# someone-in-somewhere/multimodal_rag

Hardware: AMD Instinct MI355X
Metric: chunks embedded/sec + queries/sec top_k=5 over 1M×768 at 1/2/4/8 GPUs (higher is better)
Workload: dtype f16

## Files before the change

### include/mmrag.h

```cpp
#ifndef MMRAG_H
#define MMRAG_H

#include <stddef.h>
#include <stdint.h>

#ifdef __cplusplus
extern "C" {
#endif

#define MMRAG_OK 0
#define MMRAG_EINVAL 1
#define MMRAG_EWORKSPACE 2
#define MMRAG_EHIP 3
#define MMRAG_EUNSUPPORTED 4

#define MMRAG_F32 0
#define MMRAG_F16 1
#define MMRAG_BF16 2
#define MMRAG_F8E4M3 3

#define MMRAG_MAX_K 20

int mmrag_abi_version(void);
const char *mmrag_last_error(void);

int64_t mmrag_padded_dim(int d, int dtype);

size_t mmrag_cosine_topk_workspace_bytes(int B, int64_t n, int k);

int mmrag_cosine_topk(const void *q, const void *corpus, int B, int64_t n, int d, int64_t ld,
                      int dtype, int k, int64_t row_offset, const uint32_t *alive_bits,
                      float *out_scores, int64_t *out_rows, void *workspace,
                      size_t workspace_bytes, void *stream);

int mmrag_cosine_topk_lists(const void *q, const void *corpus, int B, int64_t n, int d, int64_t ld,
                            int dtype, int k, const uint32_t *alive_bits, void *workspace,
                            size_t workspace_bytes, void *stream);
int mmrag_cosine_topk_select(int B, int64_t n, int k, int64_t row_offset, const void *workspace,
                             float *out_scores, int64_t *out_rows, void *stream);

#define MMRAG_MAX_K_DEEP 4096
size_t mmrag_cosine_topk_deep_workspace_bytes(int B, int64_t n, int k);
int mmrag_cosine_topk_deep(const void *q, const void *corpus, int B, int64_t n, int d, int64_t ld,
                           int dtype, int k, int64_t row_offset, const uint32_t *alive_bits,
                           float *out_scores, int64_t *out_rows, void *workspace,
                           size_t workspace_bytes, void *stream);

#define MMRAG_MAX_RESCORE_CANDIDATES 4096
int mmrag_rescore_topk(const void *q, const void *plane, int64_t ld, int dtype, int d, const int64_t *cand_rows,
                       int B, int C, int k, float *out_scores, int64_t *out_rows, void *stream);

int mmrag_merge_topk(const float *scores, const int64_t *rows, int G, int B, int k_in, int k,
                     float *out_scores, int64_t *out_rows, void *stream);
int mmrag_merge_topk_host(const float *scores, const int64_t *rows, int G, int B, int k_in,
                          int k, float *out_scores, int64_t *out_rows);
int mmrag_merge_topk_host_packed(const void *blocks, int G, int B, int k_in, int k,
                                 float *out_scores, int64_t *out_rows);

int mmrag_append_rows(void *corpus, int64_t capacity, int64_t ld, int dtype, int64_t n_used,
                      const float *new_rows, int64_t m, int d, void *stream);

int mmrag_gather_rows(void *dst, const void *src, int64_t ld, int dtype,
// ... 367 lines not shown
```

### multimodal_rag_amd/_native.py

```python
from __future__ import annotations

import ctypes
import os
import threading
from ctypes import c_char_p, c_float, c_int, c_int32, c_int64, c_size_t, c_void_p
from typing import Optional, Tuple

import numpy as np
import torch

_PKG = os.path.dirname(os.path.abspath(__file__))
LIB_PATH = os.path.join(_PKG, "lib", "libmmrag.so")

F32, F16, BF16, F8E4M3 = 0, 1, 2, 3
MAX_K = 20
MAX_K_DEEP = 4096
MAX_MMR_CANDIDATES = 1024
MAX_RESCORE_CANDIDATES = 4096
MAX_GROUP_CANDIDATES, MAX_GROUPS, MAX_GROUP_SIZE = 4096, 256, 16
MAX_FUSE_LISTS, MAX_FUSE_CANDIDATES, MAX_FUSE_RESULTS = 16, 256, 4096
FUSE_METHODS = {"rrf": 0, "max": 1}
MAX_JOIN_PAIRS = 1 << 26
MAX_CLUSTERS = 4096
MAX_SCOPE_GROUPS = 64
# ... 20 lines not shown
    pass


def _declare(lib):
    lib.mmrag_abi_version.restype = c_int
    lib.mmrag_last_error.restype = c_char_p
    lib.mmrag_padded_dim.restype = c_int64
    lib.mmrag_padded_dim.argtypes = [c_int, c_int]
    lib.mmrag_cosine_topk_workspace_bytes.restype = c_size_t
    lib.mmrag_cosine_topk_workspace_bytes.argtypes = [c_int, c_int64, c_int]
    lib.mmrag_cosine_topk.restype = c_int
    lib.mmrag_cosine_topk.argtypes = [c_void_p, c_void_p, c_int, c_int64, c_int, c_int64, c_int, c_int,
                                      c_int64, c_void_p, c_void_p, c_void_p, c_void_p, c_size_t, c_void_p]
    lib.mmrag_cosine_topk_lists.restype = c_int
    lib.mmrag_cosine_topk_lists.argtypes = [c_void_p, c_void_p, c_int, c_int64, c_int, c_int64, c_int, c_int,
                                            c_void_p, c_void_p, c_size_t, c_void_p]
    lib.mmrag_internal_search_uses_qs.restype = c_int
    lib.mmrag_internal_search_uses_qs.argtypes = [c_int, c_int64, c_int64, c_int, c_int]
    lib.mmrag_internal_cosine_topk_lists_ex.restype = c_int
    lib.mmrag_internal_cosine_topk_lists_ex.argtypes = [c_void_p, c_void_p, c_int, c_int64, c_int, c_int64, c_int,
                                                        c_int, c_void_p, c_void_p, c_size_t, c_void_p, ctypes.c_uint]
    lib.mmrag_cosine_topk_select.restype = c_int
    lib.mmrag_cosine_topk_select.argtypes = [c_int, c_int64, c_int, c_int64, c_void_p, c_void_p, c_void_p, c_void_p]
    lib.mmrag_cosine_topk_deep_workspace_bytes.restype = c_size_t
    lib.mmrag_cosine_topk_deep_workspace_bytes.argtypes = [c_int, c_int64, c_int]
    lib.mmrag_cosine_topk_deep.restype = c_int
    lib.mmrag_cosine_topk_deep.argtypes = lib.mmrag_cosine_topk.argtypes
    lib.mmrag_internal_cosine_topk_deep_ex.restype = c_int
    lib.mmrag_internal_cosine_topk_deep_ex.argtypes = lib.mmrag_cosine_topk.argtypes + [ctypes.c_uint, c_int64]
    lib.mmrag_rescore_topk.restype = c_int
    lib.mmrag_rescore_topk.argtypes = [c_void_p, c_void_p, c_int64, c_int, c_int, c_void_p, c_int, c_int, c_int,
                                       c_void_p, c_void_p, c_void_p]
    lib.mmrag_merge_topk.restype = c_int
    lib.mmrag_merge_topk.argtypes = [c_void_p, c_void_p, c_int, c_int, c_int, c_int, c_void_p, c_void_p, c_void_p]
    lib.mmrag_merge_topk_host.restype = c_int
    lib.mmrag_merge_topk_host.argtypes = [c_void_p, c_void_p, c_int, c_int, c_int, c_int, c_void_p, c_void_p]
    lib.mmrag_merge_topk_host_packed.restype = c_int
    lib.mmrag_merge_topk_host_packed.argtypes = [c_void_p, c_int, c_int, c_int, c_int, c_void_p, c_void_p]
    lib.mmrag_append_rows.restype = c_int
    lib.mmrag_append_rows.argtypes = [c_void_p, c_int64, c_int64, c_int, c_int64, c_void_p, c_int64, c_int, c_void_p]
    lib.mmrag_gather_rows.restype = c_int
    lib.mmrag_gather_rows.argtypes = [c_void_p, c_void_p, c_int64, c_int, c_void_p, c_int64, c_void_p]
    lib.mmrag_fetch_rows_f32.restype = c_int
    lib.mmrag_fetch_rows_f32.argtypes = [c_void_p, c_int64, c_int, c_void_p, c_int64, c_int, c_void_p, c_void_p]
    lib.mmrag_device_info.restype = c_int
    lib.mmrag_device_info.argtypes = [ctypes.POINTER(c_int), ctypes.POINTER(c_int), ctypes.POINTER(c_int64)]
# ... 321 lines not shown
    return buf[B * k * 8:].view(torch.float32).view(B, k), buf[: B * k * 8].view(torch.int64).view(B, k)


def search_uses_query_stationary(B: int, n: int, d: int, k: int, dtype: torch.dtype) -> bool:
    return bool(lib().mmrag_internal_search_uses_qs(B, n, padded_dim(d, dtype), _TORCH2DT[dtype], k))


def search_kernel_name(B: int, n: int, d: int, k: int, dtype: torch.dtype) -> str:
    v = lib().mmrag_internal_search_uses_qs(B, n, padded_dim(d, dtype), _TORCH2DT[dtype], k)
    return {0: "cosine_topk_kernel (slab-ring)", 1: "cosine_topk_qs_kernel", 2: "cosine_topk_walk_kernel"}[v]


def padded_dim(d: int, dtype: torch.dtype) -> int:
    v = lib().mmrag_padded_dim(int(d), _TORCH2DT[dtype])
    if v < 0:
        raise MMRagNativeError(f"padded_dim: bad arguments d={d} dtype={dtype}")
    return int(v)


DBG_NO_PREPASS, DBG_8_WAVES, DBG_NO_QS, DBG_FORCE_QS = 1, 2, 4, 8
DBG_OLD_QS, DBG_MFMA32, DBG_MFMA16, DBG_NO_DYN, DBG_NO_SEED = 0x10000, 0x20000, 0x40000, 0x80000, 0x100000


def cosine_topk(q: torch.Tensor, corpus: torch.Tensor, n: int, d: int, k: int, row_offset: int = 0,
                alive_bits: Optional[torch.Tensor] = None,
                workspace: Optional[torch.Tensor] = None, dbg: int = 0,
                packed_out: bool = False) -> Tuple[torch.Tensor, torch.Tensor]:
    _dev_check(q, corpus, alive_bits)
    _check_q_rows("cosine_topk", q, corpus, n)
    B, ld = q.shape
    L = lib()
    need = L.mmrag_cosine_topk_workspace_bytes(B, n, k)
    if workspace is None or _nbytes(workspace) < need:
        workspace = torch.empty(max(need, 16), dtype=torch.uint8, device=q.device)
    out_s, out_r = _topk_out(B, k, q.device, packed_out)
    if dbg:
        cosine_topk_lists(q, corpus, n, d, k, workspace, alive_bits=alive_bits, dbg=dbg)
        return cosine_topk_select(B, n, k, row_offset, workspace, out_s, out_r)
    with torch.cuda.device(q.device):
        st = L.mmrag_cosine_topk(q.data_ptr(), corpus.data_ptr(), B, n, d, ld, _TORCH2DT[q.dtype], k, row_offset,
                                 alive_bits.data_ptr() if alive_bits is not None else None,
                                 out_s.data_ptr(), out_r.data_ptr(), workspace.data_ptr(), _nbytes(workspace),
                                 _stream_ptr(q.device))
    _check(st, "mmrag_cosine_topk")
    return out_s, out_r


DEEP_DBG_NO_BOUND = 1


def cosine_topk_deep(q: torch.Tensor, corpus: torch.Tensor, n: int, d: int, k: int, row_offset: int = 0,
                     alive_bits: Optional[torch.Tensor] = None, workspace: Optional[torch.Tensor] = None,
                     dbg: int = 0, cap: int = 0) -> Tuple[torch.Tensor, torch.Tensor]:
    _dev_check(q, corpus, alive_bits)
    _check_q_rows("cosine_topk_deep", q, corpus, n)
    B, ld = q.shape
    L = lib()
    need = cosine_topk_deep_workspace_bytes(B, n, k)
    if workspace is None or _nbytes(workspace) < need:
        workspace = torch.empty(max(need, 16), dtype=torch.uint8, device=q.device)
    out_s, out_r = _topk_out(B, k, q.device)
# ... 1191 lines not shown
    with torch.cuda.device(corpus.device):
        st = lib().mmrag_fetch_rows_f32(corpus.data_ptr(), corpus.shape[1], _TORCH2DT[corpus.dtype], rows.data_ptr(),
                                        rows.numel(), d, out.data_ptr(), _stream_ptr(corpus.device))
    _check(st, "mmrag_fetch_rows_f32")
    return out


def cosine_topk_lists(q: torch.Tensor, corpus: torch.Tensor, n: int, d: int, k: int, workspace: torch.Tensor,
                      alive_bits: Optional[torch.Tensor] = None, dbg: int = 0) -> None:
    _dev_check(q, corpus, workspace, alive_bits)
    if q.dtype != corpus.dtype or q.shape[1] != corpus.shape[1] or not q.is_contiguous() or not corpus.is_contiguous():
        raise MMRagNativeError("cosine_topk_lists: q and corpus must be contiguous and share dtype and padded width")
    if n > corpus.shape[0]:
        raise MMRagNativeError(f"cosine_topk_lists: n={n} exceeds corpus capacity {corpus.shape[0]}")
    B, ld = q.shape
    with torch.cuda.device(q.device):
        st = lib().mmrag_internal_cosine_topk_lists_ex(
            q.data_ptr(), corpus.data_ptr(), B, n, d, ld, _TORCH2DT[q.dtype], k,
            alive_bits.data_ptr() if alive_bits is not None else None, workspace.data_ptr(),
            _nbytes(workspace), _stream_ptr(q.device), int(dbg))
    _check(st, "mmrag_cosine_topk_lists")


def cosine_topk_select(B: int, n: int, k: int, row_offset: int, workspace: torch.Tensor,
                       out_scores: Optional[torch.Tensor] = None,
                       out_rows: Optional[torch.Tensor] = None) -> Tuple[torch.Tensor, torch.Tensor]:
    _dev_check(workspace)
    dev = workspace.device
    if out_scores is None:
        out_scores = torch.empty((B, k), dtype=torch.float32, device=dev)
    if out_rows is None:
        out_rows = torch.empty((B, k), dtype=torch.int64, device=dev)
    with torch.cuda.device(dev):
        st = lib().mmrag_cosine_topk_select(B, n, k, row_offset, workspace.data_ptr(), out_scores.data_ptr(),
                                            out_rows.data_ptr(), _stream_ptr(dev))
    _check(st, "mmrag_cosine_topk_select")
    return out_scores, out_rows


ACT_NONE, ACT_GELU, ACT_QUICK_GELU = 0, 1, 2
ARCH_BERT, ARCH_PRELN = 0, 1
POOL_MEAN, POOL_FIRST, POOL_SELECT = 0, 1, 2


class EncoderDesc(ctypes.Structure):
    _fields_ = [("arch", c_int32), ("n_layers", c_int32), ("hidden", c_int32), ("n_heads", c_int32),
                ("intermediate", c_int32), ("vocab", c_int32), ("max_pos", c_int32), ("pool", c_int32),
                ("act", c_int32), ("causal", c_int32), ("normalize", c_int32), ("out_dim", c_int32),
                ("ln_eps", c_float), ("image", c_int32), ("patch", c_int32)]


def _ptr(t: Optional[torch.Tensor]):
    return t.data_ptr() if t is not None else None


def linear_f16(x: torch.Tensor, wt: torch.Tensor, bias: Optional[torch.Tensor] = None, act: int = ACT_NONE,
               resid: Optional[torch.Tensor] = None, out: Optional[torch.Tensor] = None) -> torch.Tensor:
    _dev_check(x, wt, bias, resid, out)
# ... 561 lines not shown
        raise MMRagNativeError("copy_to_host_async: need a host destination at least as large as the device source")
    _check(lib().mmrag_copy_to_host_async(dst_host.data_ptr(), src_dev.data_ptr(), nbytes, stream),
           "mmrag_copy_to_host_async")


class SearchPlan:

    def __init__(self, q: torch.Tensor, corpus: torch.Tensor, n: int, d: int, k: int, workspace: torch.Tensor,
                 alive_bits: Optional[torch.Tensor] = None):
        _dev_check(q, corpus, workspace, alive_bits)
        if q.dtype != corpus.dtype or q.shape[1] != corpus.shape[1] or not q.is_contiguous() or not corpus.is_contiguous():
            raise MMRagNativeError("SearchPlan: q and corpus must be contiguous and share dtype and padded width")
        if n > corpus.shape[0]:
            raise MMRagNativeError(f"SearchPlan: n={n} exceeds corpus capacity {corpus.shape[0]}")
        need = lib().mmrag_cosine_topk_workspace_bytes(q.shape[0], n, k)
        if _nbytes(workspace) < need:
            raise MMRagNativeError("SearchPlan: workspace too small")
        self._keep = (q, corpus, workspace, alive_bits)
        self.B, self.n, self.k = q.shape[0], n, k
        self._scan_args = (q.data_ptr(), corpus.data_ptr(), q.shape[0], n, d, q.shape[1], _TORCH2DT[q.dtype], k,
                           alive_bits.data_ptr() if alive_bits is not None else None, workspace.data_ptr(),
                           _nbytes(workspace))
        self._ws = workspace.data_ptr()
        self._scan = lib().mmrag_cosine_topk_lists
        self._select = lib().mmrag_cosine_topk_select

    def scan(self, stream: int) -> None:
        st = self._scan(*self._scan_args, stream)
        if st:
            _check(st, "mmrag_cosine_topk_lists")

    def select(self, row_offset: int, out_scores_ptr: int, out_rows_ptr: int, stream: int) -> None:
        st = self._select(self.B, self.n, self.k, row_offset, self._ws, out_scores_ptr, out_rows_ptr, stream)
        if st:
            _check(st, "mmrag_cosine_topk_select")
```

### multimodal_rag_amd/csrc/search.hip

```cpp
#include "slab_ring.h"

#include <stdlib.h>

using namespace mmrag;

namespace mmrag_impl {

template <int DT, int WN, int K, int NSTAGE, int NW, bool SEEDED>
__global__ __launch_bounds__(64 * NW, NW / 4) void cosine_topk_kernel(const KParams p) {
#if defined(__HIP_DEVICE_COMPILE__)
#include "slab_ring_body.inc"
#endif
}

template <int K>
struct FullList {
    float v[K];
    long long r[K];
    __device__ inline void init() {
#pragma unroll
        for (int i = 0; i < K; ++i) {
            v[i] = NEG_INF;
            r[i] = LLONG_MAX;
        }
    }
    __device__ inline void insert(float x, long long xr) {
#pragma unroll
        for (int j = 0; j < K; ++j) {
            const bool b = better(x, xr, v[j], r[j]);
            const float nv = b ? x : v[j];
            const float nx = b ? v[j] : x;
            const long long nr = b ? xr : r[j];
            const long long nxr = b ? r[j] : xr;
            v[j] = nv;
            x = nx;
            r[j] = nr;
            xr = nxr;
        }
    }
    __device__ inline void pop() {
#pragma unroll
        for (int j = 0; j + 1 < K; ++j) {
            v[j] = v[j + 1];
            r[j] = r[j + 1];
        }
        v[K - 1] = NEG_INF;
        r[K - 1] = LLONG_MAX;
    }
};

template <int K>
__device__ inline void wave_extract(FullList<K> &l, float *out_v, long long *out_r) {
#pragma unroll
    for (int round = 0; round < K; ++round) {
        float s = l.v[0];
        long long r = l.r[0];
#pragma unroll
        for (int off = 32; off >= 1; off >>= 1) {
            const float os = __shfl_xor(s, off);
            const long long orr = __shfl_xor(r, off);
            if (better(os, orr, s, r)) {
                s = os;
                r = orr;
            }
        }
        out_v[round] = s;
        out_r[round] = r;
        if (l.v[0] == s && l.r[0] == r) l.pop();
    }
}
// ... 39 lines not shown
        for (int i = lane; i < 4 * K; i += 64)
            if (sh_r[i] != LLONG_MAX) l.insert(sh_v[i], sh_r[i]);
        wave_extract<K>(l, ov, orr);
        if (lane == 0) {
#pragma unroll
            for (int i = 0; i < K; ++i) {
                if (i < k_out) {
                    const bool valid = orr[i] != LLONG_MAX && ov[i] > NEG_INF;
                    out_s[(size_t)q * k_out + i] = valid ? ov[i] : NEG_INF;
                    out_r[(size_t)q * k_out + i] = valid ? orr[i] + row_offset : -1;
                }
            }
            if (thr0 != nullptr) {
                const bool full = orr[K - 1] != LLONG_MAX && ov[K - 1] > NEG_INF;
                thr0[q] = full ? ov[K - 1] : NEG_INF;
#pragma unroll
                for (int i = 0; i < K; ++i) {
                    const bool valid = orr[i] != LLONG_MAX && ov[i] > NEG_INF;
                    seed_s[(size_t)q * seed_q_stride + i] = valid ? ov[i] : NEG_INF;
                    seed_r[(size_t)q * seed_q_stride + i] = valid ? (int)orr[i] : INT_MAX;
                }
            }
        }
    }
}

struct Plan {
    int K;
    int WN;
    int NW;
    int grid_x, grid_y;
    int n_tiles;
    int n_lists;
    int b_pad;
    int pre_tiles;
    bool qs_ok;
    bool qs_room;
};

constexpr unsigned DBG_NO_PREPASS = 1u, DBG_8_WAVES = 2u, DBG_NO_QS = 4u, DBG_FORCE_QS = 8u;
constexpr unsigned DBG_OLD_QS = 0x10000u, DBG_MFMA32 = 0x20000u, DBG_MFMA16 = 0x40000u, DBG_NO_DYN = 0x80000u,
                   DBG_NO_SEED = 0x100000u;

Plan make_plan(int B, long long n, int k, unsigned dbg = 0) {
    Plan pl;
    pl.K = k <= 5 ? 5 : (k <= 10 ? 10 : 20);
// ... 62 lines not shown
    const dim3 grid(grid_x, grid_y);
    with_elem_type(dtype, [&](auto tag) { launch_filter<decltype(tag)::value>(WN, p, grid, s); });
    MMRAG_CHECK_HIP(hipGetLastError());
    return MMRAG_OK;
}

template <typename RowT>
int launch_merge(int K, const float *cs, const RowT *cr, long long n_cand, long long inner,
                 long long outer_stride, long long q_stride, int B, int k_out, long long row_offset,
                 float *out_s, long long *out_r, hipStream_t s, float *thr0 = nullptr, float *seed_s = nullptr,
                 int *seed_r = nullptr, long long seed_q_stride = 0) {
    if (K == 5)
        merge_topk_kernel<5, RowT><<<B, 256, 0, s>>>(cs, cr, n_cand, inner, outer_stride, q_stride, k_out,
                                                     row_offset, out_s, out_r, thr0, seed_s, seed_r, seed_q_stride);
    else if (K == 10)
        merge_topk_kernel<10, RowT><<<B, 256, 0, s>>>(cs, cr, n_cand, inner, outer_stride, q_stride, k_out,
                                                      row_offset, out_s, out_r, thr0, seed_s, seed_r, seed_q_stride);
    else
        merge_topk_kernel<20, RowT><<<B, 256, 0, s>>>(cs, cr, n_cand, inner, outer_stride, q_stride, k_out,
                                                      row_offset, out_s, out_r, thr0, seed_s, seed_r, seed_q_stride);
    return MMRAG_OK;
}

__global__ void fill_empty_kernel(float *s, long long *r, long long total) {
    const long long i = (long long)blockIdx.x * blockDim.x + threadIdx.x;
    if (i < total) {
        s[i] = NEG_INF;
        r[i] = -1;
    }
}

__global__ void fill_seed_empty_kernel(float *s, int *r, long long q_stride, int K, long long n_queries) {
    const long long q = (long long)blockIdx.x * blockDim.x + threadIdx.x;
    if (q < n_queries)
        for (int i = 0; i < K; ++i) {
            s[q * q_stride + i] = NEG_INF;
            r[q * q_stride + i] = INT_MAX;
        }
}

int check_search_args(const char *name, int k_max, const void *q, const void *corpus, int B, int64_t n, int d, int64_t ld,
                      int dtype, int k) {
    MMRAG_CHECK_ARG(dtype >= 0 && dtype <= MMRAG_F8E4M3, "%s: bad dtype %d", name, dtype);
    MMRAG_CHECK_ARG(B > 0, "%s: B must be positive (got %d)", name, B);
    MMRAG_CHECK_ARG(k >= 1 && k <= k_max, "%s: k=%d outside 1..%d", name, k, k_max);
    MMRAG_CHECK_ARG(n >= 0 && n < (int64_t)INT_MAX - TM, "%s: n=%lld out of range", name, (long long)n);
// ... 14 lines not shown

extern "C" {

struct WsLayout {
    size_t entries, off_r, off_thr, off_ts, off_tr, off_cnt, cnt_bytes, off_pub, off_pthr, off_tk, xch_end, total;
};
static WsLayout ws_layout(const Plan &pl) {
    WsLayout w;
    w.entries = (size_t)pl.b_pad * pl.n_lists * pl.K;
    w.off_r = w.entries * sizeof(float);
    w.off_thr = w.off_r + w.entries * sizeof(int);
    w.off_ts = w.off_thr + (size_t)pl.b_pad * sizeof(float);
    w.off_tr = (w.off_ts + (size_t)pl.b_pad * pl.K * sizeof(float) + 15) / 16 * 16;
    w.off_cnt = (w.off_tr + (size_t)pl.b_pad * pl.K * sizeof(long long) + 63) / 64 * 64;
    w.cnt_bytes = 0;
    w.off_pub = w.off_cnt + w.cnt_bytes;
    w.off_pthr = w.off_pub + (pl.qs_room ? (size_t)pl.b_pad * pl.grid_x * sizeof(float) : 0);
    w.off_tk = w.off_pthr + (pl.qs_room ? (size_t)pl.b_pad * sizeof(float) : 0);
    w.xch_end = w.off_tk + (pl.qs_room ? ((size_t)pl.grid_y * sizeof(unsigned) + 63) / 64 * 64 : 0);
    w.total = w.xch_end;
    return w;
}

size_t mmrag_cosine_topk_workspace_bytes(int B, int64_t n, int k) {
    if (B <= 0 || n < 0 || k < 1 || k > MMRAG_MAX_K) return 0;
    return ws_layout(make_plan(B, n, k)).total + 256;
}

int mmrag_internal_cosine_topk_lists_ex(const void *q, const void *corpus, int B, int64_t n, int d, int64_t ld,
                                        int dtype, int k, const uint32_t *alive_bits, void *workspace,
                                        size_t workspace_bytes, void *stream, unsigned dbg) {
    if (int st = check_search_args("cosine_topk", MMRAG_MAX_K, q, corpus, B, n, d, ld, dtype, k)) return st;
    if (n == 0) return MMRAG_OK;
    const Plan pl = make_plan(B, n, k, dbg);
    const WsLayout wl = ws_layout(pl);
    if (!workspace || workspace_bytes < wl.total) {
        set_error("cosine_topk: workspace %zu bytes < required %zu", workspace_bytes, wl.total);
        return MMRAG_EWORKSPACE;
    }
    MMRAG_CHECK_ARG(((uintptr_t)workspace % 16) == 0, "cosine_topk: workspace must be 16-byte aligned");

    KParams p;
    p.q = (const char *)q;
    p.corpus = (const char *)corpus;
    p.alive_bits = alive_bits;
    p.cand_s = (float *)workspace;
    p.cand_r = (int *)((char *)workspace + wl.off_r);
    p.n = n;
    p.B = B;
    p.row_bytes = (unsigned)(ld * esize(dtype));
    p.n_tiles = pl.n_tiles;
    p.n_lists = pl.n_lists;
    p.tile0 = 0;
    p.thr0 = nullptr;
    p.dbg = dbg;
    p.stamps = ((dbg & DBG_QS_CLOCK) && workspace_bytes >= wl.total + 256 * (size_t)(pl.grid_x * pl.grid_y)) ? (unsigned long long *)((char *)workspace + wl.total) : nullptr;
    p.walkers = pl.grid_x;
    p.share_l2 = pl.grid_y > 1;
    p.sample_best = nullptr;
    p.pub_best = nullptr;
    p.pub_thr = nullptr;
    p.tickets = nullptr;
    p.p_static = INT_MAX / 2;
    hipStream_t s = (hipStream_t)stream;
    const size_t seed_off = (size_t)(pl.n_lists - 1) * pl.K;
    const int walk_mfma = (dbg & DBG_MFMA32) ? 32 : ((dbg & DBG_MFMA16) ? 16 : (pl.K == 5 ? QSW_DEFAULT_MFMA : 32));
    if (pl.qs_ok && !(dbg & DBG_OLD_QS) && qsw_supported(dtype, p.row_bytes, pl.K, walk_mfma)) {
        const int tiles = (int)((n + QS_TILE_ROWS - 1) / QS_TILE_ROWS);
        const int per = tiles / pl.grid_x;
        p.n_tiles = tiles;
        p.pub_best = nullptr;
        p.pub_thr = nullptr;
        p.tickets = nullptr;
        p.p_static = INT_MAX / 2;
        const bool seed = per >= 12 && !(dbg & DBG_NO_SEED);
        const bool dyn = pl.grid_y == 1 && per >= 24 && !(dbg & DBG_NO_DYN);
        if (seed || dyn) {
            MMRAG_CHECK_HIP(hipMemsetD32Async((hipDeviceptr_t)((char *)workspace + wl.off_pub), (int)TICKET0,
                                              (wl.xch_end - wl.off_pub) / 4, s));
            if (seed) {
                p.pub_best = (float *)((char *)workspace + wl.off_pub);
                p.pub_thr = (float *)((char *)workspace + wl.off_pthr);
            }
            if (dyn) {
                p.tickets = (unsigned *)((char *)workspace + wl.off_tk);
                const int tail = per / 10 > 3 ? per / 10 : 3;
                p.p_static = per - tail;
            }
        }
        if (int st = qsw_launch(dtype, pl.K, walk_mfma, p, pl.grid_x, pl.grid_y, s)) return st;
        MMRAG_CHECK_HIP(hipGetLastError());
        return MMRAG_OK;
    }
    if (pl.qs_ok && qs_supported(dtype, p.row_bytes, pl.K)) {
        const int tiles = (int)((n + QS_TILE_ROWS - 1) / QS_TILE_ROWS);
        float *thr0 = nullptr;
        if (pl.pre_tiles > 0) {
            KParams ks = p;
            ks.n_tiles = pl.pre_tiles * (TM / QS_TILE_ROWS);
            ks.sample_best = (float *)((char *)workspace + wl.off_pub);
            if (int st = qs_launch(dtype, pl.K, ks, pl.grid_x, pl.grid_y, s)) return st;
            thr0 = (float *)((char *)workspace + wl.off_thr);
// ... 29 lines not shown
        MMRAG_CHECK_HIP(hipGetLastError());
        if (int st = run(pre, pl.n_tiles - pre, pl.grid_x, thr0)) return st;
    } else {
        if (pl.n_lists > pl.grid_x) {
            const long long total = (long long)pl.b_pad;
            fill_seed_empty_kernel<<<(unsigned)((total + 255) / 256), 256, 0, s>>>(
                p.cand_s + seed_off, p.cand_r + seed_off, (long long)pl.n_lists * pl.K, pl.K, total);
        }
        if (int st = run(0, pl.n_tiles, pl.grid_x, nullptr)) return st;
    }
    MMRAG_CHECK_HIP(hipGetLastError());
    return MMRAG_OK;
}

int mmrag_internal_search_uses_qs(int B, int64_t n, int64_t ld, int dtype, int k) {
    if (B <= 0 || n <= 0 || k <= 0 || k > MMRAG_MAX_K) return 0;
    const Plan pl = make_plan(B, n, k, 0u);
    const unsigned rb = (unsigned)(ld * esize(dtype));
    if (!pl.qs_ok) return 0;
    if (qsw_supported(dtype, rb, pl.K, QSW_DEFAULT_MFMA)) return 2;
    return qs_supported(dtype, rb, pl.K) ? 1 : 0;
}

int mmrag_cosine_topk_lists(const void *q, const void *corpus, int B, int64_t n, int d, int64_t ld, int dtype,
                            int k, const uint32_t *alive_bits, void *workspace, size_t workspace_bytes,
                            void *stream) {
    return mmrag_internal_cosine_topk_lists_ex(q, corpus, B, n, d, ld, dtype, k, alive_bits, workspace,
                                               workspace_bytes, stream, 0u);
}

int mmrag_cosine_topk_select(int B, int64_t n, int k, int64_t row_offset, const void *workspace,
                             float *out_scores, int64_t *out_rows, void *stream) {
    MMRAG_CHECK_ARG(B > 0 && n >= 0 && k >= 1 && k <= MMRAG_MAX_K, "cosine_topk_select: bad shape");
    MMRAG_CHECK_ARG(out_scores && out_rows, "cosine_topk_select: null output");
    hipStream_t s = (hipStream_t)stream;
    if (n == 0) {
        const long long total = (long long)B * k;
        fill_empty_kernel<<<(unsigned)((total + 255) / 256), 256, 0, s>>>(out_scores, (long long *)out_rows, total);
        MMRAG_CHECK_HIP(hipGetLastError());
        return MMRAG_OK;
    }
    MMRAG_CHECK_ARG(workspace, "cosine_topk_select: null workspace");
    const Plan pl = make_plan(B, n, k);
    const WsLayout wl = ws_layout(pl);
    const float *cand_s = (const float *)workspace;
    const int *cand_r = (const int *)((const char *)workspace + wl.off_r);
    const long long n_cand = (long long)pl.n_lists * pl.K;
    launch_merge<int>(pl.K, cand_s, cand_r, n_cand, n_cand, 0, n_cand, B, k, row_offset, out_scores,
                      (long long *)out_rows, s);
    MMRAG_CHECK_HIP(hipGetLastError());
    return MMRAG_OK;
}

int mmrag_cosine_topk(const void *q, const void *corpus, int B, int64_t n, int d, int64_t ld, int dtype,
                      int k, int64_t row_offset, const uint32_t *alive_bits, float *out_scores,
                      int64_t *out_rows, void *workspace, size_t workspace_bytes, void *stream) {
    if (int st = mmrag_cosine_topk_lists(q, corpus, B, n, d, ld, dtype, k, alive_bits, workspace, workspace_bytes,
                                         stream))
        return st;
    return mmrag_cosine_topk_select(B, n, k, row_offset, workspace, out_scores, out_rows, stream);
}

int mmrag_merge_topk(const float *scores, const int64_t *rows, int G, int B, int k_in, int k,
                     float *out_scores, int64_t *out_rows, void *stream) {
    MMRAG_CHECK_ARG(scores && rows && out_scores && out_rows, "merge_topk: null pointer");
    MMRAG_CHECK_ARG(G > 0 && B > 0 && k_in > 0, "merge_topk: bad shape G=%d B=%d k_in=%d", G, B, k_in);
    MMRAG_CHECK_ARG(k >= 1 && k <= MMRAG_MAX_K, "merge_topk: k=%d outside 1..%d", k, MMRAG_MAX_K);
    const int K = k <= 5 ? 5 : (k <= 10 ? 10 : 20);
    launch_merge<long long>(K, scores, (const long long *)rows, (long long)G * k_in, k_in, (long long)B * k_in,
                            k_in, B, k, 0, out_scores, (long long *)out_rows, (hipStream_t)stream);
    MMRAG_CHECK_HIP(hipGetLastError());
    return MMRAG_OK;
}

// ... 2 lines not shown
```

### multimodal_rag_amd/index.py

```python
from __future__ import annotations

import gc
import logging
import operator
import threading
import time
from collections import OrderedDict
from typing import Any, Callable, Dict, List, Optional, Sequence, Tuple

import numpy as np
import torch

from . import _native
from .boost import BoostSpec, check_prior_values
from .filters import ColumnRegistry, names_added_at, pack_programs, try_compile
from .hostutil import load_hostrows
from .tracing import stage

_HOSTROWS = load_hostrows()

logger = logging.getLogger(__name__)


_CMP: Dict[str, Callable[[Any, Any], bool]] = {
# ... 134 lines not shown
        self.name = name
        self.metadata = dict(metadata or {})
        self.dim = int(dim)
        self.dtype = dtype
        self.device = torch.device(device)
        self.ld = _native.padded_dim(self.dim, dtype)
        cap = max(int(capacity), 256)
        self._matrix = self._new_rows(cap, zero=True)
        self.plane_ld = _native.padded_dim(self.dim, rescore_dtype) if rescore_dtype is not None else 0
        self._plane: Optional[torch.Tensor] = None
        if rescore_dtype is not None:
            self._plane = torch.zeros((cap, self.plane_ld), dtype=rescore_dtype, device=self.device)
        self._alive_dev = torch.zeros(self._n_words(cap), dtype=torch.int32, device=self.device)
        self._alive_host = np.zeros(self._n_words(cap), dtype=np.uint32)
        self._n = 0
        self._n_dead = 0
        self._ids: List[Optional[str]] = []
        self._documents: List[Optional[str]] = []
        self._metadatas: List[Dict[str, Any]] = []
        self._meta_index = MetaIndex()
        self._row_of: Dict[str, int] = {}
        self._lock = threading.RLock()
        self._search_ws: Optional[torch.Tensor] = None
        self._deep_ws: Optional[torch.Tensor] = None
        self._scoped_ws: Optional[torch.Tensor] = None
        self._lex = None
        self._sparse = None
        self._pending_sparse = None
        self._groups: Dict[str, Dict[str, Any]] = {}
        self._boosted_ws: Optional[torch.Tensor] = None
        self._recommend_ws: Optional[torch.Tensor] = None
        self._added_at = np.full(cap, np.nan, dtype=np.float64)
        self._priors: Dict[str, Any] = {}
        self._spec_cols: "OrderedDict[Tuple[str, float], Dict[str, Any]]" = OrderedDict()
        self.f32_exact = bool(settings.MMRAG_F32_EXACT_SEARCH)
        self._filter_cols = ColumnRegistry(lambda: (self._metadatas, self._n, self._added_at))
        self._filtered_ws: Optional[torch.Tensor] = None
        self._range_ws: Optional[torch.Tensor] = None
        self.device_filters = bool(settings.MMRAG_DEVICE_FILTERS)
        self._tokens = None
        self._late_ws: Optional[torch.Tensor] = None

    def _new_rows(self, rows: int, zero: bool) -> torch.Tensor:
        make = torch.zeros if zero else torch.empty
        if self.is_f8:
            return make((rows, self.ld), dtype=torch.uint8, device=self.device).view(torch.float8_e4m3fn)
# ... 495 lines not shown
    def _launch_search_rescored(self, query_embeddings, n_results: int, where, check_norm: bool):
        from .config import settings

        qf = self._to_device_f32(query_embeddings, "query", check_norm)
        q8 = self._pack_queries(qf, check_norm=False)
        qp = self._pack_plane_queries(qf)
        bits = self._where_bits(where)
        if n_results <= _native.MAX_K_DEEP:
            C = min(max(_native.MAX_K, int(settings.MMRAG_F8_OVERSAMPLE) * n_results), _native.MAX_K_DEEP)
            C = max(C, n_results)
            _, cand = self._scan(q8, C, bits)
            return _native.rescore_topk(qp, self._plane, self.dim, cand.contiguous(), n_results, packed_out=True)
        scores, rows = self._scan(q8, n_results, bits)
        return _cat_pairs([_native.rescore_topk(qp, self._plane, self.dim, rows[:, i:i + _native.MAX_K].contiguous(),
                                                min(_native.MAX_K, rows.shape[1] - i))
                           for i in range(0, rows.shape[1], _native.MAX_K)], 1)

    def _scan(self, q: torch.Tensor, n_results: int, bits):
        if n_results <= _native.MAX_K and self.f32_exact and self.dtype == torch.float32 and q.shape[0] > 64:
            return self._in_slices(q, 64, lambda qi: _native.cosine_topk(qi, self._matrix, self._n, self.dim, n_results,
                                                                         alive_bits=bits))
        if n_results <= _native.MAX_K:
            need = _native.cosine_topk_workspace_bytes(q.shape[0], self._n, n_results)
            return _native.cosine_topk(q, self._matrix, self._n, self.dim, n_results, alive_bits=bits,
                                       workspace=self._workspace("_search_ws", need), packed_out=True)
        if n_results <= _native.MAX_K_DEEP:
            step = 64 if self.f32_exact and self.dtype == torch.float32 else q.shape[0]

            def deep(qi: torch.Tensor):
                need = _native.cosine_topk_deep_workspace_bytes(qi.shape[0], self._n, n_results)
                return _native.cosine_topk_deep(qi, self._matrix, self._n, self.dim, n_results, alive_bits=bits,
                                                workspace=self._workspace("_deep_ws", need))

            return self._in_slices(q, step, deep)
        if q.shape[0] != 1:
            raise ValueError(f"n_results > {_native.MAX_K_DEEP} is supported for single queries only")
        if bits is None:
            bits = self._alive_dev
        bits = bits.clone()
        out_s, out_r, left = [], [], n_results
        while left > 0:
            k = min(left, _native.MAX_K)
            s, r = _native.cosine_topk(q, self._matrix, self._n, self.dim, k, alive_bits=bits)
            out_s.append(s)
            out_r.append(r)
            got = r[0]
            got = got[got >= 0]
            if got.numel() < k:
                break
            host = got.cpu().numpy()
            w = bits.cpu().numpy().view(np.uint32).copy()
            np.bitwise_and.at(w, host >> 5, ~(np.uint32(1) << (host & 31).astype(np.uint32)))
            bits = torch.from_numpy(w.view(np.int32)).to(self.device)
            left -= k
        return torch.cat(out_s, 1), torch.cat(out_r, 1)

    def _workspace(self, name: str, need: int) -> Optional[torch.Tensor]:
        if torch.cuda.current_stream(self.device) != torch.cuda.default_stream(self.device):
            return None
        ws = getattr(self, name)
        if ws is None or ws.numel() < need:
            ws = torch.empty(max(need, 16), dtype=torch.uint8, device=self.device)
            setattr(self, name, ws)
        return ws

    @staticmethod
    def _in_slices(q: torch.Tensor, step: int, run):
        return _cat_pairs([run(q[i:i + step]) for i in range(0, q.shape[0], step)], 0)

    def search(self, query_embeddings, n_results: int, where: Optional[Dict[str, Any]] = None):
        with self._lock:
            return self._launch_search(query_embeddings, n_results, where)

    def _tables(self):
        return self._ids, self._documents, self._metadatas

    @staticmethod
    def _rows_of(tables, rows: Sequence[int], include: Sequence[str]):
        ids_t, docs_t, metas_t = tables
        return ([ids_t[r] for r in rows],
                [docs_t[r] for r in rows] if "documents" in include else None,
                [dict(metas_t[r]) for r in rows] if "metadatas" in include else None)

    @classmethod
    def _append_hits(cls, out: Dict[str, Any], tables, rows: Sequence[int], include: Sequence[str]):
        for key, col in zip(("ids", "documents", "metadatas"), cls._rows_of(tables, rows, include)):
# ... 1525 lines not shown
```

Before: 692,300.

## Fuse exchange-buffer rearm into new select kernel and skip per-search memset

Adds a dedicated per-query top-k select kernel that uses 32-bit row ids and wave-shuffle reduction, replacing the generic merge launch. It also re-initialises the scan's seed/exchange buffer with ticket values at the end of select. A host-side state token records that the buffer is already armed, so the next scan can skip its hipMemsetD32Async. This removes one memset launch per search and a slower merge, at the cost of host-side state that must be reset whenever the workspace is reallocated or reused by another caller.

```diff
diff --git a/include/mmrag.h b/include/mmrag.h
--- a/include/mmrag.h
+++ b/include/mmrag.h
@@ -38,6 +38,15 @@
                             size_t workspace_bytes, void *stream);
 int mmrag_cosine_topk_select(int B, int64_t n, int k, int64_t row_offset, const void *workspace,
                              float *out_scores, int64_t *out_rows, void *stream);
+
+typedef struct {
+    uint64_t armed;
+} mmrag_scan_state;
+int mmrag_cosine_topk_lists_s(const void *q, const void *corpus, int B, int64_t n, int d, int64_t ld,
+                              int dtype, int k, const uint32_t *alive_bits, void *workspace,
+                              size_t workspace_bytes, mmrag_scan_state *state, void *stream);
+int mmrag_cosine_topk_select_s(int B, int64_t n, int k, int64_t row_offset, void *workspace,
+                               float *out_scores, int64_t *out_rows, mmrag_scan_state *state, void *stream);
 
 #define MMRAG_MAX_K_DEEP 4096
 size_t mmrag_cosine_topk_deep_workspace_bytes(int B, int64_t n, int k);
diff --git a/multimodal_rag_amd/_native.py b/multimodal_rag_amd/_native.py
--- a/multimodal_rag_amd/_native.py
+++ b/multimodal_rag_amd/_native.py
@@ -66,6 +66,18 @@
                                                         c_int, c_void_p, c_void_p, c_size_t, c_void_p, ctypes.c_uint]
     lib.mmrag_cosine_topk_select.restype = c_int
     lib.mmrag_cosine_topk_select.argtypes = [c_int, c_int64, c_int, c_int64, c_void_p, c_void_p, c_void_p, c_void_p]
+    lib.mmrag_cosine_topk_lists_s.restype = c_int
+    lib.mmrag_cosine_topk_lists_s.argtypes = [c_void_p, c_void_p, c_int, c_int64, c_int, c_int64, c_int, c_int,
+                                              c_void_p, c_void_p, c_size_t, c_void_p, c_void_p]
+    lib.mmrag_cosine_topk_select_s.restype = c_int
+    lib.mmrag_cosine_topk_select_s.argtypes = [c_int, c_int64, c_int, c_int64, c_void_p, c_void_p, c_void_p, c_void_p,
+                                               c_void_p]
+    lib.mmrag_internal_cosine_topk_select_ex.restype = c_int
+    lib.mmrag_internal_cosine_topk_select_ex.argtypes = [c_int, c_int64, c_int, c_int64, c_void_p, c_void_p, c_void_p,
+                                                         c_void_p, c_void_p, ctypes.c_uint]
+    lib.mmrag_internal_exchange_range.restype = c_int
+    lib.mmrag_internal_exchange_range.argtypes = [c_int, c_int64, c_int, ctypes.POINTER(c_size_t),
+                                                  ctypes.POINTER(c_size_t)]
     lib.mmrag_cosine_topk_deep_workspace_bytes.restype = c_size_t
     lib.mmrag_cosine_topk_deep_workspace_bytes.argtypes = [c_int, c_int64, c_int]
     lib.mmrag_cosine_topk_deep.restype = c_int
@@ -433,10 +445,24 @@
 DBG_OLD_QS, DBG_MFMA32, DBG_MFMA16, DBG_NO_DYN, DBG_NO_SEED = 0x10000, 0x20000, 0x40000, 0x80000, 0x100000
 
 
+class ScanState(ctypes.Structure):
+    _fields_ = [("armed", ctypes.c_uint64)]
+
+    def reset(self) -> None:
+        self.armed = 0
+
+
+def exchange_range(B: int, n: int, k: int) -> Tuple[int, int]:
+    off, length = c_size_t(0), c_size_t(0)
+    _check(lib().mmrag_internal_exchange_range(B, n, k, ctypes.byref(off), ctypes.byref(length)),
+           "mmrag_internal_exchange_range")
+    return off.value, length.value
+
+
 def cosine_topk(q: torch.Tensor, corpus: torch.Tensor, n: int, d: int, k: int, row_offset: int = 0,
                 alive_bits: Optional[torch.Tensor] = None,
                 workspace: Optional[torch.Tensor] = None, dbg: int = 0,
-                packed_out: bool = False) -> Tuple[torch.Tensor, torch.Tensor]:
+                packed_out: bool = False, state: Optional[ScanState] = None) -> Tuple[torch.Tensor, torch.Tensor]:
     _dev_check(q, corpus, alive_bits)
     _check_q_rows("cosine_topk", q, corpus, n)
     B, ld = q.shape
@@ -444,10 +470,26 @@
     need = L.mmrag_cosine_topk_workspace_bytes(B, n, k)
     if workspace is None or _nbytes(workspace) < need:
         workspace = torch.empty(max(need, 16), dtype=torch.uint8, device=q.device)
+        if state is not None:
+            state.reset()
     out_s, out_r = _topk_out(B, k, q.device, packed_out)
     if dbg:
+        if state is not None:
+            state.reset()
         cosine_topk_lists(q, corpus, n, d, k, workspace, alive_bits=alive_bits, dbg=dbg)
         return cosine_topk_select(B, n, k, row_offset, workspace, out_s, out_r)
+    if state is not None:
+        sp = ctypes.addressof(state)
+        with torch.cuda.device(q.device):
+            stream = _stream_ptr(q.device)
+            st = L.mmrag_cosine_topk_lists_s(q.data_ptr(), corpus.data_ptr(), B, n, d, ld, _TORCH2DT[q.dtype], k,
+                                             alive_bits.data_ptr() if alive_bits is not None else None,
+                                             workspace.data_ptr(), _nbytes(workspace), sp, stream)
+            _check(st, "mmrag_cosine_topk_lists_s")
+            st = L.mmrag_cosine_topk_select_s(B, n, k, row_offset, workspace.data_ptr(), out_s.data_ptr(),
+                                              out_r.data_ptr(), sp, stream)
+        _check(st, "mmrag_cosine_topk_select_s")
+        return out_s, out_r
     with torch.cuda.device(q.device):
         st = L.mmrag_cosine_topk(q.data_ptr(), corpus.data_ptr(), B, n, d, ld, _TORCH2DT[q.dtype], k, row_offset,
                                  alive_bits.data_ptr() if alive_bits is not None else None,
@@ -1685,9 +1727,13 @@
     _check(st, "mmrag_cosine_topk_lists")
 
 
+SELECT_DBG_OLD_MERGE = 1
+
+
 def cosine_topk_select(B: int, n: int, k: int, row_offset: int, workspace: torch.Tensor,
                        out_scores: Optional[torch.Tensor] = None,
-                       out_rows: Optional[torch.Tensor] = None) -> Tuple[torch.Tensor, torch.Tensor]:
+                       out_rows: Optional[torch.Tensor] = None, state: Optional[ScanState] = None,
+                       dbg: int = 0) -> Tuple[torch.Tensor, torch.Tensor]:
     _dev_check(workspace)
     dev = workspace.device
     if out_scores is None:
@@ -1695,8 +1741,9 @@
     if out_rows is None:
         out_rows = torch.empty((B, k), dtype=torch.int64, device=dev)
     with torch.cuda.device(dev):
-        st = lib().mmrag_cosine_topk_select(B, n, k, row_offset, workspace.data_ptr(), out_scores.data_ptr(),
-                                            out_rows.data_ptr(), _stream_ptr(dev))
+        st = lib().mmrag_internal_cosine_topk_select_ex(
+            B, n, k, row_offset, workspace.data_ptr(), out_scores.data_ptr(), out_rows.data_ptr(),
+            ctypes.addressof(state) if state is not None else None, _stream_ptr(dev), int(dbg))
     _check(st, "mmrag_cosine_topk_select")
     return out_scores, out_rows
 
@@ -2304,15 +2351,18 @@
                            alive_bits.data_ptr() if alive_bits is not None else None, workspace.data_ptr(),
                            _nbytes(workspace))
         self._ws = workspace.data_ptr()
-        self._scan = lib().mmrag_cosine_topk_lists
-        self._select = lib().mmrag_cosine_topk_select
+        self.state = ScanState()
+        self._state = ctypes.addressof(self.state)
+        self._scan = lib().mmrag_cosine_topk_lists_s
+        self._select = lib().mmrag_cosine_topk_select_s
 
     def scan(self, stream: int) -> None:
-        st = self._scan(*self._scan_args, stream)
+        st = self._scan(*self._scan_args, self._state, stream)
         if st:
-            _check(st, "mmrag_cosine_topk_lists")
+            _check(st, "mmrag_cosine_topk_lists_s")
 
     def select(self, row_offset: int, out_scores_ptr: int, out_rows_ptr: int, stream: int) -> None:
-        st = self._select(self.B, self.n, self.k, row_offset, self._ws, out_scores_ptr, out_rows_ptr, stream)
+        st = self._select(self.B, self.n, self.k, row_offset, self._ws, out_scores_ptr, out_rows_ptr, self._state,
+                          stream)
         if st:
-            _check(st, "mmrag_cosine_topk_select")
+            _check(st, "mmrag_cosine_topk_select_s")
diff --git a/multimodal_rag_amd/csrc/search.hip b/multimodal_rag_amd/csrc/search.hip
--- a/multimodal_rag_amd/csrc/search.hip
+++ b/multimodal_rag_amd/csrc/search.hip
@@ -13,25 +13,26 @@
 #endif
 }
 
-template <int K>
+template <int K, typename RowT = long long>
 struct FullList {
+    static constexpr RowT PAD = sizeof(RowT) == 4 ? (RowT)INT_MAX : (RowT)LLONG_MAX;
     float v[K];
-    long long r[K];
+    RowT r[K];
     __device__ inline void init() {
 #pragma unroll
         for (int i = 0; i < K; ++i) {
             v[i] = NEG_INF;
-            r[i] = LLONG_MAX;
-        }
-    }
-    __device__ inline void insert(float x, long long xr) {
+            r[i] = PAD;
+        }
+    }
+    __device__ inline void insert(float x, RowT xr) {
 #pragma unroll
         for (int j = 0; j < K; ++j) {
             const bool b = better(x, xr, v[j], r[j]);
             const float nv = b ? x : v[j];
             const float nx = b ? v[j] : x;
-            const long long nr = b ? xr : r[j];
-            const long long nxr = b ? r[j] : xr;
+            const RowT nr = b ? xr : r[j];
+            const RowT nxr = b ? r[j] : xr;
             v[j] = nv;
             x = nx;
             r[j] = nr;
@@ -45,7 +46,7 @@
             r[j] = r[j + 1];
         }
         v[K - 1] = NEG_INF;
-        r[K - 1] = LLONG_MAX;
+        r[K - 1] = PAD;
     }
 };
 
@@ -131,6 +132,71 @@
                 }
             }
         }
+    }
+}
+
+constexpr int SELECT_QPB = 4, SELECT_LOADS = 8;
+
+template <int K>
+__global__ __launch_bounds__(64 * SELECT_QPB) void select_topk_kernel(const float *__restrict__ cs,
+                                                                      const int *__restrict__ cr, int n_cand, int B,
+                                                                      int k_out, long long row_offset,
+                                                                      float *__restrict__ out_s,
+                                                                      long long *__restrict__ out_r,
+                                                                      uint4 *__restrict__ rearm, unsigned rearm_words) {
+    const int lane = threadIdx.x & 63;
+    const int q = blockIdx.x * SELECT_QPB + (threadIdx.x >> 6);
+    if (q < B) {
+        const float *qs = cs + (size_t)q * n_cand;
+        const int *qr = cr + (size_t)q * n_cand;
+        FullList<K, int> l;
+        l.init();
+        for (int c0 = lane; c0 < n_cand; c0 += 64 * SELECT_LOADS) {
+            float s[SELECT_LOADS];
+            int r[SELECT_LOADS];
+#pragma unroll
+            for (int u = 0; u < SELECT_LOADS; ++u) {
+                const int c = c0 + 64 * u;
+                s[u] = c < n_cand ? qs[c] : NEG_INF;
+                r[u] = c < n_cand ? qr[c] : INT_MAX;
+            }
+#pragma unroll
+            for (int u = 0; u < SELECT_LOADS; ++u)
+                if (r[u] != INT_MAX && r[u] >= 0 && better(s[u], r[u], l.v[K - 1], l.r[K - 1])) l.insert(s[u], r[u]);
+        }
+        float my_s = NEG_INF;
+        int my_r = INT_MAX;
+#pragma unroll
+        for (int round = 0; round < K; ++round) {
+            float s = l.v[0];
+            int r = l.r[0];
+#pragma unroll
+            for (int off = 32; off >= 1; off >>= 1) {
+                const float os = __shfl_xor(s, off);
+                const int orr = __shfl_xor(r, off);
+                if (better(os, orr, s, r)) {
+                    s = os;
+                    r = orr;
+                }
+            }
+            if (lane == round) {
+                my_s = s;
+                my_r = r;
+            }
+            if (l.v[0] == s && l.r[0] == r) l.pop();
+        }
+        if (lane < k_out) {
+            const bool valid = my_r != INT_MAX && my_s > NEG_INF;
+            out_s[(size_t)q * k_out + lane] = valid ? my_s : NEG_INF;
+            out_r[(size_t)q * k_out + lane] = valid ? (long long)my_r + row_offset : -1;
+        }
+    }
+    if (rearm != nullptr) {
+        const unsigned per = (rearm_words + gridDim.x - 1) / gridDim.x;
+        const unsigned lo = blockIdx.x * per;
+        const unsigned hi = lo + per < rearm_words ? lo + per : rearm_words;
+        for (unsigned i = lo + threadIdx.x; i < hi; i += 64 * SELECT_QPB)
+            rearm[i] = make_uint4(TICKET0, TICKET0, TICKET0, TICKET0);
     }
 }
 
@@ -239,6 +305,20 @@
     return MMRAG_OK;
 }
 
+void launch_select(int K, const float *cs, const int *cr, int n_cand, int B, int k_out, long long row_offset,
+                   float *out_s, long long *out_r, uint4 *rearm, unsigned rearm_words, hipStream_t s) {
+    const unsigned grid = (unsigned)((B + SELECT_QPB - 1) / SELECT_QPB);
+    if (K == 5)
+        select_topk_kernel<5><<<grid, 64 * SELECT_QPB, 0, s>>>(cs, cr, n_cand, B, k_out, row_offset, out_s, out_r,
+                                                               rearm, rearm_words);
+    else if (K == 10)
+        select_topk_kernel<10><<<grid, 64 * SELECT_QPB, 0, s>>>(cs, cr, n_cand, B, k_out, row_offset, out_s, out_r,
+                                                                rearm, rearm_words);
+    else
+        select_topk_kernel<20><<<grid, 64 * SELECT_QPB, 0, s>>>(cs, cr, n_cand, B, k_out, row_offset, out_s, out_r,
+                                                                rearm, rearm_words);
+}
+
 __global__ void fill_empty_kernel(float *s, long long *r, long long total) {
     const long long i = (long long)blockIdx.x * blockDim.x + threadIdx.x;
     if (i < total) {
@@ -299,14 +379,20 @@
     return w;
 }
 
+static uint64_t exchange_token(const WsLayout &wl) {
+    return (1ull << 63) | ((uint64_t)(wl.off_pub / 64) << 28) | (uint64_t)((wl.xch_end - wl.off_pub) / 64);
+}
+
 size_t mmrag_cosine_topk_workspace_bytes(int B, int64_t n, int k) {
     if (B <= 0 || n < 0 || k < 1 || k > MMRAG_MAX_K) return 0;
     return ws_layout(make_plan(B, n, k)).total + 256;
 }
 
-int mmrag_internal_cosine_topk_lists_ex(const void *q, const void *corpus, int B, int64_t n, int d, int64_t ld,
-                                        int dtype, int k, const uint32_t *alive_bits, void *workspace,
-                                        size_t workspace_bytes, void *stream, unsigned dbg) {
+static int lists_impl(const void *q, const void *corpus, int B, int64_t n, int d, int64_t ld, int dtype, int k,
+                      const uint32_t *alive_bits, void *workspace, size_t workspace_bytes, mmrag_scan_state *state,
+                      void *stream, unsigned dbg) {
+    const uint64_t armed = state ? state->armed : 0;
+    if (state) state->armed = 0;
     if (int st = check_search_args("cosine_topk", MMRAG_MAX_K, q, corpus, B, n, d, ld, dtype, k)) return st;
     if (n == 0) return MMRAG_OK;
     const Plan pl = make_plan(B, n, k, dbg);
@@ -353,8 +439,9 @@
         const bool seed = per >= 12 && !(dbg & DBG_NO_SEED);
         const bool dyn = pl.grid_y == 1 && per >= 24 && !(dbg & DBG_NO_DYN);
         if (seed || dyn) {
-            MMRAG_CHECK_HIP(hipMemsetD32Async((hipDeviceptr_t)((char *)workspace + wl.off_pub), (int)TICKET0,
-                                              (wl.xch_end - wl.off_pub) / 4, s));
+            if (armed != exchange_token(wl))
+                MMRAG_CHECK_HIP(hipMemsetD32Async((hipDeviceptr_t)((char *)workspace + wl.off_pub), (int)TICKET0,
+                                                  (wl.xch_end - wl.off_pub) / 4, s));
             if (seed) {
                 p.pub_best = (float *)((char *)workspace + wl.off_pub);
                 p.pub_thr = (float *)((char *)workspace + wl.off_pthr);
@@ -430,15 +517,36 @@
     return qs_supported(dtype, rb, pl.K) ? 1 : 0;
 }
 
+int mmrag_internal_cosine_topk_lists_ex(const void *q, const void *corpus, int B, int64_t n, int d, int64_t ld,
+                                        int dtype, int k, const uint32_t *alive_bits, void *workspace,
+                                        size_t workspace_bytes, void *stream, unsigned dbg) {
+    return lists_impl(q, corpus, B, n, d, ld, dtype, k, alive_bits, workspace, workspace_bytes, nullptr, stream, dbg);
+}
+
+int mmrag_cosine_topk_lists_s(const void *q, const void *corpus, int B, int64_t n, int d, int64_t ld, int dtype,
+                              int k, const uint32_t *alive_bits, void *workspace, size_t workspace_bytes,
+                              mmrag_scan_state *state, void *stream) {
+    return lists_impl(q, corpus, B, n, d, ld, dtype, k, alive_bits, workspace, workspace_bytes, state, stream, 0u);
+}
+
 int mmrag_cosine_topk_lists(const void *q, const void *corpus, int B, int64_t n, int d, int64_t ld, int dtype,
                             int k, const uint32_t *alive_bits, void *workspace, size_t workspace_bytes,
                             void *stream) {
-    return mmrag_internal_cosine_topk_lists_ex(q, corpus, B, n, d, ld, dtype, k, alive_bits, workspace,
-                                               workspace_bytes, stream, 0u);
-}
-
-int mmrag_cosine_topk_select(int B, int64_t n, int k, int64_t row_offset, const void *workspace,
-                             float *out_scores, int64_t *out_rows, void *stream) {
+    return lists_impl(q, corpus, B, n, d, ld, dtype, k, alive_bits, workspace, workspace_bytes, nullptr, stream, 0u);
+}
+
+int mmrag_internal_exchange_range(int B, int64_t n, int k, size_t *off, size_t *len) {
+    MMRAG_CHECK_ARG(B > 0 && n > 0 && k >= 1 && k <= MMRAG_MAX_K && off && len, "exchange_range: bad arguments");
+    const WsLayout wl = ws_layout(make_plan(B, n, k));
+    *off = wl.off_pub;
+    *len = wl.xch_end - wl.off_pub;
+    return MMRAG_OK;
+}
+
+constexpr unsigned SELECT_DBG_OLD_MERGE = 1u;
+int mmrag_internal_cosine_topk_select_ex(int B, int64_t n, int k, int64_t row_offset, void *workspace,
+                                         float *out_scores, int64_t *out_rows, mmrag_scan_state *state, void *stream,
+                                         unsigned dbg) {
     MMRAG_CHECK_ARG(B > 0 && n >= 0 && k >= 1 && k <= MMRAG_MAX_K, "cosine_topk_select: bad shape");
     MMRAG_CHECK_ARG(out_scores && out_rows, "cosine_topk_select: null output");
     hipStream_t s = (hipStream_t)stream;
@@ -454,10 +562,32 @@
     const float *cand_s = (const float *)workspace;
     const int *cand_r = (const int *)((const char *)workspace + wl.off_r);
     const long long n_cand = (long long)pl.n_lists * pl.K;
-    launch_merge<int>(pl.K, cand_s, cand_r, n_cand, n_cand, 0, n_cand, B, k, row_offset, out_scores,
-                      (long long *)out_rows, s);
+    if (dbg & SELECT_DBG_OLD_MERGE) {
+        launch_merge<int>(pl.K, cand_s, cand_r, n_cand, n_cand, 0, n_cand, B, k, row_offset, out_scores,
+                          (long long *)out_rows, s);
+        MMRAG_CHECK_HIP(hipGetLastError());
+        if (state) state->armed = 0;
+        return MMRAG_OK;
+    }
+    const bool rearm = state != nullptr && pl.qs_room;
+    if (rearm) MMRAG_CHECK_ARG(((uintptr_t)workspace % 16) == 0, "cosine_topk_select: workspace must be 16-byte aligned");
+    launch_select(pl.K, cand_s, cand_r, (int)n_cand, B, k, row_offset, out_scores, (long long *)out_rows,
+                  rearm ? (uint4 *)((char *)workspace + wl.off_pub) : nullptr,
+                  rearm ? (unsigned)((wl.xch_end - wl.off_pub) / 16) : 0u, s);
     MMRAG_CHECK_HIP(hipGetLastError());
-    return MMRAG_OK;
+    if (state) state->armed = rearm ? exchange_token(wl) : 0;
+    return MMRAG_OK;
+}
+
+int mmrag_cosine_topk_select_s(int B, int64_t n, int k, int64_t row_offset, void *workspace, float *out_scores,
+                               int64_t *out_rows, mmrag_scan_state *state, void *stream) {
+    return mmrag_internal_cosine_topk_select_ex(B, n, k, row_offset, workspace, out_scores, out_rows, state, stream, 0u);
+}
+
+int mmrag_cosine_topk_select(int B, int64_t n, int k, int64_t row_offset, const void *workspace,
+                             float *out_scores, int64_t *out_rows, void *stream) {
+    return mmrag_internal_cosine_topk_select_ex(B, n, k, row_offset, (void *)workspace, out_scores, out_rows, nullptr,
+                                                stream, 0u);
 }
 
 int mmrag_cosine_topk(const void *q, const void *corpus, int B, int64_t n, int d, int64_t ld, int dtype,
diff --git a/multimodal_rag_amd/index.py b/multimodal_rag_amd/index.py
--- a/multimodal_rag_amd/index.py
+++ b/multimodal_rag_amd/index.py
@@ -180,6 +180,7 @@
         self._row_of: Dict[str, int] = {}
         self._lock = threading.RLock()
         self._search_ws: Optional[torch.Tensor] = None
+        self._search_state = _native.ScanState()
         self._deep_ws: Optional[torch.Tensor] = None
         self._scoped_ws: Optional[torch.Tensor] = None
         self._lex = None
@@ -721,8 +722,9 @@
                                                                          alive_bits=bits))
         if n_results <= _native.MAX_K:
             need = _native.cosine_topk_workspace_bytes(q.shape[0], self._n, n_results)
-            return _native.cosine_topk(q, self._matrix, self._n, self.dim, n_results, alive_bits=bits,
-                                       workspace=self._workspace("_search_ws", need), packed_out=True)
+            ws = self._workspace("_search_ws", need)
+            return _native.cosine_topk(q, self._matrix, self._n, self.dim, n_results, alive_bits=bits, workspace=ws,
+                                       packed_out=True, state=self._search_state if ws is not None else None)
         if n_results <= _native.MAX_K_DEEP:
             step = 64 if self.f32_exact and self.dtype == torch.float32 else q.shape[0]
 
@@ -761,6 +763,8 @@
         if ws is None or ws.numel() < need:
             ws = torch.empty(max(need, 16), dtype=torch.uint8, device=self.device)
             setattr(self, name, ws)
+            if name == "_search_ws":
+                self._search_state.reset()
         return ws
 
     @staticmethod
```

New measurement: 702,100, median of 6. +1.4%, better.
